# QueensGambit/CrazyAra

Hardware: AMD Instinct MI355X
Metric: nn_evals_per_sec (higher is better)
Workload: dtype f16x3; 1 GPU; crazyhouse RISEv2 19-block (34x8x8 planes -> 5184 policy + value), batch=256, inputs resident in HBM, random-init seeded weights; batch=256, parallelism=replicas x1, precision=float16x3

## Files before the change

### crazyara_amd/csrc/nn/kernels.h

```cpp
#pragma once
#include <hip/hip_runtime.h>
#include <cstdint>

namespace cra {

typedef _Float16 half_t;

constexpr int kSquares = 64;

inline int64_t packed_weight_elems(int cout_pad, int k_total) { return int64_t(cout_pad) * k_total; }

struct ConvArgs {
    const void* x;
    const void* wpk;
    const void* wpk_lo;
    const float* bias;
    const void* resid;
    void* out;
    int batch;
    int cin;
    int cout_pad;
    int cout_real;
    int cout_ld;
    int ks;
    int relu;
    int out_policy_f32;
    int out_flat;
    int flat_pitch;
    int out_rows_f32;
    int rows_valid;
    float* softmax_out;
    const float* planes;
    int planes_c;
    int p8;
    float acc_scale;
    const void *pre_wpk, *pre_wpk_lo;
    const float* pre_bias;
    float pre_acc_scale;
    int dev;
    int few_boards;
    int x_ld;
};

template <typename T> void launch_conv_gemm(const ConvArgs& a, hipStream_t s);

struct BlockArgs {
    const void* x;
    void* y;
    const void* w1pk;
    const float* b1;
    const float* wdw;
    const float* b2;
    const void* w3pk;
    const void* w1pk_lo;
    const void* w3pk_lo;
    const float* b3;
    int batch, C, cop_pad, ks;
    const float* gate;
    float* pool_out;
    const float* dwpk;
};
template <typename T> void launch_block(const BlockArgs& a, hipStream_t s);
void launch_conv_gemm_x3(const ConvArgs& a, hipStream_t s);
void launch_block_x3(const BlockArgs& a, hipStream_t s);
void init_x3_kernel_attributes();
int block_x3_chunk_channels();
struct X3TowerBlock {
    const void *w1pk, *w1pk_lo, *w3pk, *w3pk_lo;
    const float* dwpk;
    const float* b3;
    const float* se_w1t;
    const float* se_w2t;
    const float* se_b;
    int cop_pad;
    int se_kind;
    float w1_inv, w3_scale, w3_inv;
    int tail;
};
static_assert(sizeof(X3TowerBlock) == 96, "the tower kernels index a device array of these");
struct X3TowerArgs {
    const float* x;
    float* y;
    const X3TowerBlock* blocks;
    int nblocks;
    int batch;
    int p8;
    int ks;
    int symmetric;
    int no_tail;
    int no_quad;
};
void launch_tower_x3(const X3TowerArgs& a, hipStream_t s);
const char* tower_x3_kernel_name(const X3TowerArgs& a);
void launch_tower_x3_tail(const X3TowerArgs& a, hipStream_t s);
void init_x3_tail_kernel_attributes();
void launch_tower_x3_quad(const X3TowerArgs& a, hipStream_t s);
void init_x3_quad_kernel_attributes();
bool block_x3w_supports(int C, int ks);
void launch_block_x3w(const BlockArgs& a, hipStream_t s);
void init_x3_wblock_kernel_attributes();
void launch_se_gate_w(const float* pool, float* gate, int kind, const float* w1t, const float* w2t, const float* b1, int batch, int C, hipStream_t s);
constexpr int kX3WSplitMaxG = 8;
struct X3WSplitArgs {
    BlockArgs blk;
    const float* x_parts;
    float* y_parts;
    int gin, G;
    int stream_in;
};
int x3w_split_chunks(int cop_pad);
int x3w_split_shares(int cop_pad, int boards, int cu_count);
void launch_block_x3w_split(const X3WSplitArgs& a, hipStream_t s);
void launch_x3w_split_finish(const float* parts, int gin, float* y, float* pool_out, int batch, int C, hipStream_t s);
void init_x3_wsplit_kernel_attributes();
struct X3WTowerBlock {
    const void *w1pk, *w1pk_lo, *w3pk, *w3pk_lo;
    const float* dwpk;
    const float* b3;
    int cop_pad, ks;
};
static_assert(sizeof(X3WTowerBlock) == 56, "tower_x3w_kernel indexes a device array of these");
struct X3WTowerArgs {
    const float* x;
    float* y;
    const X3WTowerBlock* blocks;
    int nblocks;
    const float* gate;
    float* pool_out;
    int batch, C;
};
bool tower_x3w_supports(int C, int ks);
void launch_tower_x3w(const X3WTowerArgs& a, hipStream_t s);
void init_x3_wtower_kernel_attributes();
struct NtbLayer {
    const void *wh, *wl;
    const float* bias;
};
struct NtbArgs {
    const float* x;
    float* y;
    int batch, C, D, M, H;
    NtbLayer patch, qkv, proj, projection, mhca, mhca_proj, mlp1, mlp2;
};
bool ntb_x3w_supports(int C, int D, int M, int H);
void launch_ntb_x3w(const NtbArgs& a, hipStream_t s);
void init_x3_wntb_kernel_attributes();
struct X3SplitArgs {
    X3TowerBlock blk;
    const float* x_parts;
    float* y_parts;
    int gin;
    int batch, G;
    const float* pool_in;
    float* pool_out;
    int dev;
};
void launch_block_x3_split(const X3SplitArgs& a, hipStream_t s);
void launch_x3_split_finish(const float* parts, int gin, float* y, int batch, hipStream_t s);
template <typename T> void init_block_kernel_attributes();
template <typename T> int block_chunk_channels();

constexpr int kTowerWindow = 16;
struct TowerBlockDesc {
    const float* b3;
    const float* s3;
    const void* se_w1;
    const void* se_w2;
    const float* se_b;
    int cop_pad;
    int ks;
    int se_kind;
    float qx_inv, qt_inv, escale;
};
// ... 164 lines not shown
```

### crazyara_amd/csrc/nn/precision.cpp

```cpp
#include <cstdlib>
#include <stdexcept>

#include "rise_net.h"

namespace cra {

namespace {
constexpr bool kX3ValueHeadOneLaunch = true;
}

RiseNet::DevSwitches::DevSwitches() {
    if (const char* e = getenv("CRA_X3_CONV_DEV")) conv_dev = atoi(e);
    device_graph = getenv("CRA_DEVICE_GRAPH") != nullptr;
    lane_graph = getenv("CRA_LANE_GRAPH") != nullptr;
    lane_no_graph = getenv("CRA_LANE_NO_GRAPH") != nullptr;
    predict_copy = getenv("CRA_PREDICT_COPY") != nullptr;
    predict_zero_copy = getenv("CRA_PREDICT_ZERO_COPY") != nullptr;
    if (const char* e = getenv("CRA_LANE_LAUNCHES")) lane_launches = e[0];
    lane_sync = getenv("CRA_LANE_SYNC") != nullptr;
    if (const char* e = getenv("CRA_X3_TOWER")) x3_symmetric = e[0] == 's';
    if (const char* e = getenv("CRA_X3_SPLIT_DEV")) x3_split_dev = atoi(e);
    no_small_path = getenv("CRA_NO_SMALL_PATH") != nullptr;
    if (const char* e = getenv("CRA_SMALL_BATCH_CONV_SPLIT")) small_conv_split = atoi(e);
    tower_trace = getenv("CRA_TOWER_TRACE") != nullptr;
    x3_value_one_launch = kX3ValueHeadOneLaunch;
    if (const char* e = getenv("CRA_X3_VALUE_HEAD")) x3_value_one_launch = e[0] == 'o';
    value_head_debug = getenv("CRA_VALUE_HEAD_DEBUG") != nullptr;
    if (const char* e = getenv("CRA_VALUE_HEAD_LDS_PAD")) value_head_lds_pad = atoi(e);
    if (const char* e = getenv("CRA_VALUE_HEAD_VARIANT")) value_head_variant = atoi(e);
    x3_no_head_chain = getenv("CRA_X3_NO_HEAD_CHAIN") != nullptr;
    x3_no_tail = getenv("CRA_X3_NO_TAIL") != nullptr;
    x3_no_quad = getenv("CRA_X3_NO_QUAD") != nullptr;
    small_batch_heads_apart = getenv("CRA_SMALL_BATCH_HEADS_APART") != nullptr;
}

Precision parse_precision(const std::string& precision) {
    Precision v;
    std::string prec = precision;
    auto strip = [&](const std::string& tag) {
        if (prec.size() <= tag.size() || prec.compare(prec.size() - tag.size(), tag.size(), tag) != 0) return false;
        prec.resize(prec.size() - tag.size());
        return true;
    };
    if (strip("-3k")) v.one_launch = false;
    if (strip("-8w")) v.thin_waves = true;
    if (strip("-1wg")) v.board_split = false;
    if (strip("-1b")) v.boards_per_wg = 1;
    else if (strip("-2b")) v.boards_per_wg = 2;
    if (strip("-wtower")) v.wtower = v.wnet = v.wblock = true;
    else if (strip("-wsplit")) v.wsplit = v.wnet = v.wblock = true;
    else if (strip("-wnet")) v.wnet = v.wblock = true;
    else if (strip("-wblock")) v.wblock = true;
    if (strip("-unfused")) v.fused = v.tower = false;
    else if (strip("-perblock")) v.tower = false;
    using M = Precision::Mode;
    static const std::pair<const char*, M> kModes[] = {
        {"float16", M::Float16},   {"fp16", M::Float16},     {"half", M::Float16},      {"int8", M::Int8},
        {"fp8", M::Fp8},           {"float8", M::Fp8},       {"float32", M::Float32},   {"fp32", M::Float32},
        {"float16x3", M::Float16x3}, {"fp16x3", M::Float16x3}, {"f16x3", M::Float16x3},
        {"float16p8", M::Float16p8}, {"fp16p8", M::Float16p8}, {"f16p8", M::Float16p8}};
    for (const auto& m : kModes)
        if (prec == m.first) {
            v.mode = m.second;
            if (v.wtower && !v.x3()) throw std::invalid_argument("`-wtower` is a float16x3 kernel family (float16x3-wtower | float16p8-wtower), got '" + precision + "'");
            if (v.wtower && !v.fused) throw std::invalid_argument("`-wtower` and `-unfused` exclude each other, got '" + precision + "'");
            if (v.wsplit && !v.x3()) throw std::invalid_argument("`-wsplit` is a float16x3 kernel family (float16x3-wsplit | float16p8-wsplit), got '" + precision + "'");
            if (v.wsplit && !v.fused) throw std::invalid_argument("`-wsplit` and `-unfused` exclude each other, got '" + precision + "'");
            if (v.wsplit && !v.board_split)
                throw std::invalid_argument("`-wsplit` and `-1wg` exclude each other (several workgroups per board against one), got '" + precision + "'");
            if (v.wnet && !v.x3()) throw std::invalid_argument("`-wnet` is a float16x3 kernel family (float16x3-wnet | float16p8-wnet), got '" + precision + "'");
            if (v.wnet && !v.fused) throw std::invalid_argument("`-wnet` and `-unfused` exclude each other, got '" + precision + "'");
            if (v.wblock && !v.x3()) throw std::invalid_argument("`-wblock` is a float16x3 kernel family (float16x3-wblock | float16p8-wblock), got '" + precision + "'");
            if (v.wblock && !v.fused) throw std::invalid_argument("`-wblock` and `-unfused` exclude each other, got '" + precision + "'");
            return v;
        }
    throw std::invalid_argument("unsupported precision '" + precision + "' (float16 | float16x3 | float16p8 | float32 | fp8 | int8)");
}

}
```

### crazyara_amd/csrc/nn/rise_net.h

```cpp
#pragma once
#include <hip/hip_runtime.h>
#include <memory>
#include <string>
#include <utility>
#include <vector>

#include "board_net.h"
#include "netfile.h"

namespace cra {

uint8_t float_to_e4m3(float v);
uint8_t float_to_e5m2(float v);

struct Precision {
    enum class Mode { Float32, Float16, Float16x3, Float16p8, Fp8, Int8 };
    Mode mode = Mode::Float16;
    bool fused = true;
    bool tower = true;
    bool one_launch = true;
    bool thin_waves = false;
    bool board_split = true;
    bool wblock = false;
    bool wnet = false;
// ... 27 lines not shown
        const int* board_of = nullptr;
        int n = 0;
        int layout = 0;
        const void* descs = nullptr;
        const float* planes = nullptr;
        const uint16_t* idx = nullptr;
        const uint32_t* cnt = nullptr;
        uint32_t stride = 0;
        float* gathered = nullptr;
        float* probs = nullptr;
        float* logits = nullptr;
        float* value = nullptr;
        float* aux = nullptr;
    };
    void run_group(const Group& g);

    std::vector<std::pair<float, float>> calibration_maxima(const float* planes_host, int n_boards);

    void keep_logits(bool on) override;
    void* enable_block_dump(int* n_tiles);
    void dev_launch_op(int op, int iters);
    float* value_head_debug() const { return value_head_dbg_; }
    int dev_screen_prepare();
    long dev_screen_run(int op, int launches, long* words);
    std::string dev_screen_info(int op) const;
    void forward_async();

    int launches_per_forward() const { return launches_; }
    const char* op_name(int i) const;
    const char* op_kernel(int i) const;
    void time_ops(int iters, float* ms);
    float time_forward(int iters);

    struct IoOverride {
        const float* planes = nullptr;
        float* value = nullptr;
        float* probs = nullptr;
        float* aux = nullptr;
    };
    bool last_submit_was_zero_copy() const { return last_zero_copy_; }

private:
    friend class ExpertSet;
    struct ForwardCall {
        int boards = 0;
        const IoOverride* io = nullptr;
        int prev_g = 1;
    };
    RiseNet(const std::string& model_path, int device_id, int batch_size, const std::string& precision, const RiseNet* parent);
    struct Impl;
    template <typename T> struct Builder;
    template <typename T> void build(const NetFile& nf);
    template <typename T> void enqueue(hipStream_t s, ForwardCall call);
    template <typename T> void launch_op(int i, hipStream_t s, ForwardCall& call);
    void launch_forward_in_stream(ForwardCall call);
    void forward_on(hipStream_t s, ForwardCall call);
    int boards_of_call(int n_valid) const;
    void capture();
    bool buffers_are_pinned(const float* in_planes, float* value, float* probs, float* aux);
    bool last_zero_copy_ = false;
    bool counted_in_flight_ = false;
    int staged_calls_left_ = 0;
    struct DevSwitches {
        int conv_dev = -1;
        bool device_graph = false;
        bool lane_graph = false;
        bool lane_no_graph = false;
        bool predict_copy = false;
        bool predict_zero_copy = false;
        char lane_launches = 0;
        bool lane_sync = false;
        bool x3_symmetric = false;
        int x3_split_dev = 0;
        bool no_small_path = false;
        int small_conv_split = 2;
        bool tower_trace = false;
        bool x3_value_one_launch;
        bool value_head_debug = false;
        int value_head_lds_pad = -1;
        int value_head_variant = 0;
        bool x3_no_head_chain = false;
        bool x3_no_tail = false;
        bool x3_no_quad = false;
        bool small_batch_heads_apart = false;
        DevSwitches();
    } dev_;
    float* value_head_dbg_ = nullptr;

    std::string model_file_path_;
    Precision prec_;
    std::vector<std::pair<float, float>> int8_calib_;
    static constexpr int kBoardSplitMaxBatch = 64;
    std::unique_ptr<RiseNet> small_;
    bool owns_stream_ = true;
    int stream_slot_ = -1;
    std::string precision_arg_;
    int cu_count_ = 256;
    int launches_ = 0;
    hipGraph_t graph_ = nullptr;
    hipGraphExec_t graph_exec_ = nullptr;
    void* d_desc_ = nullptr;
    std::unique_ptr<Impl> impl_;
};

std::string int8_calibration_path(const std::string& model_file_path);
std::vector<std::pair<float, float>> read_int8_calibration(const std::string& model_file_path);
std::string calibrate_int8(const std::string& model_path, int device_id, const float* planes_host, int n_boards);
std::vector<float> default_calibration_planes(int channels, int version, int* n_boards);

}
```

### crazyara_amd/csrc/nn/rise_net_build.hip

```cpp
#include <algorithm>
#include <cmath>
#include <cstring>
#include <type_traits>

#include "../chess/planes_host.h"
#include "pack.h"
#include "rise_net_impl.h"

namespace cra {

namespace {
enum class Family {
    Tower,
    X3Tower,
    X3Split,
    Fused,
    WBlock,
    WSplit,
    WTower,
    Layers,
    Transformer,
    WNtb
};
struct BlockPlan {
// ... 645 lines not shown
    ++wntb_ops;
    prod_op = -1;
    std::swap(cur, nxt);
}

template <typename T> void RiseNet::Builder<T>::flush_tower() {
    if (tower_blocks.empty()) return;
    Op op;
    op.kind = OpKind::Tower;
    op.tw.x = cur;
    op.tw.y = nxt;
    op.tw.blocks = im.upload(tower_blocks);
    op.tw.nblocks = int(tower_blocks.size());
    const TowerImage ti = close_tower_streams(std::move(tower_streams), prec.fp8_tower());
    tower_streams = TowerStreams();
    if (prec.fp8_tower()) {
        op.tw.fp8 = prec.int8() ? 2 : 1;
        op.tw.wstream_e_frags = ti.e_frags;
        op.tw.wstream = im.upload(ti.w8);
    } else {
        op.tw.wstream = im.upload(ti.w);
    }
    op.tw.bstream = im.upload(ti.b);
    op.tw.pstream = im.upload(ti.p);
    op.tw.wstream_wave_frags = ti.w_wave_frags;
    op.tw.bstream_wave_floats = ti.b_wave_floats;
    op.tw.pstream_wave_bytes = ti.p_wave_bytes;
    op.tw.batch = B;
    op.tw.gate_in = tower_gate;
    if (dev.tower_trace) op.tw.trace = static_cast<unsigned long long*>(im.dalloc(2 * 256 * sizeof(unsigned long long)));
    prod_op = int(im.ops.size());
    im.ops.push_back(op);
    tower_blocks.clear();
    tower_gate = nullptr;
    std::swap(cur, nxt);
}

template <typename T> void RiseNet::Builder<T>::flush_x3_run() {
    if (x3_blocks.empty()) return;
    if (x3_split && x3_run_ks == 3) {
        if (!split_parts[0])
            for (auto& q : split_parts) q = static_cast<float*>(im.dalloc(size_t(B) * kSplitMaxG * kSquares * C * sizeof(float)));
        const int max_g = std::max(1, std::min(int(kSplitMaxG), net.cu_count_ / B));
        const int nb = int(x3_blocks.size());
        int gin = 1;
        for (int k = 0; k < nb; ++k) {
            Op op;
            op.kind = OpKind::BlockX3Split;
            op.xs.blk = x3_blocks[k];
            op.xs.x_parts = k == 0 ? reinterpret_cast<const float*>(cur) : split_parts[k % 2];
            op.xs.y_parts = split_parts[(k + 1) % 2];
            op.xs.gin = gin;
            op.xs.batch = B;
            op.xs.G = std::min(max_g, x3_blocks[k].cop_pad / block_x3_chunk_channels());
            op.xs.dev = dev.x3_split_dev;
            if (k > 0 && x3_blocks[k].se_kind != 0 && !(dev.x3_split_dev & 8)) {
                float* pools = static_cast<float*>(im.dalloc(size_t(B) * kSplitMaxG * C * sizeof(float)));
                im.ops.back().xs.pool_out = pools;
                op.xs.pool_in = pools;
            }
            gin = op.xs.G;
            im.ops.push_back(op);
        }
        Op fin;
        fin.kind = OpKind::X3SplitFinish;
        fin.xs.x_parts = split_parts[nb % 2];
        fin.xs.gin = gin;
        fin.xs.batch = B;
        fin.xs_y = reinterpret_cast<float*>(nxt);
        im.ops.push_back(fin);
    } else {
        Op op;
        op.kind = OpKind::TowerX3;
        op.tx.x = reinterpret_cast<const float*>(cur);
        op.tx.y = reinterpret_cast<float*>(nxt);
        op.tx.blocks = im.upload(x3_blocks);
        op.tx.nblocks = int(x3_blocks.size());
        op.tx.batch = B;
        op.tx.p8 = prec.p8() ? 1 : 0;
        op.tx.ks = x3_run_ks;
        op.tx.symmetric = dev.x3_symmetric ? 1 : 0;
        op.tx.no_tail = dev.x3_no_tail ? 1 : 0;
        op.tx.no_quad = dev.x3_no_quad ? 1 : 0;
        im.ops.push_back(op);
    }
    x3_blocks.clear();
    prod_op = -1;
    std::swap(cur, nxt);
}

template <typename T> void RiseNet::Builder<T>::one_launch_head() {
    const Folded fv = fold_bn(nf, "value_head.body.0", "value_head.body.1");
    const HeadStreams hs = pack_head(fold_bn(nf, "policy_head.body.0", "policy_head.body.1"), fold_bn(nf, "policy_head.body.3", ""), fv, C, cv, cp);
    Op op;
    op.kind = OpKind::Head;
    HeadArgs& h = op.hd;
    h.x = cur;
    h.logits = net.d_logits_;
    h.probs = net.d_probs_;
    h.value = net.d_value_;
    h.aux = net.d_aux_;
    h.s1 = im.upload(hs.s1);
    h.b1 = im.upload(hs.b1);
    h.s2 = im.upload(hs.s2);
    h.s1_wave_frags = 9 * 16 + 16 + 16;
    h.s2_wave_frags = 18 * 3 + 9;
    h.vconv_bias = im.upload_d2f(fv.b, 8);
    h.cp = cp;
    h.batch = B;
    if (dev.tower_trace) h.trace = static_cast<unsigned long long*>(im.dalloc(64 * sizeof(unsigned long long)));
    const int nfl = kSquares * cv;
    if (wdl) {
        h.fc1_w = im.upload(pack_value_wdl(nf, nfl, 512));
        const float* bw = nf.get("value_head.body_wdl.0.bias").data;
        h.wdl_b[0] = bw[0]; h.wdl_b[1] = bw[1]; h.wdl_b[2] = bw[2];
        h.wdl_b[3] = nf.get("value_head.body_plys.0.bias").data[0];
        h.wdlp = 1;
        macs += 4.0 * nfl;
    } else {
        const TensorView& w2 = nf.get("value_head.body_final.2.weight");
        const float* bb = nf.get("value_head.body_final.0.bias").data;
        h.fc1_w = im.upload(pack_value_fc1_threads(nf, nfl, fc));
        h.fc1_b = im.upload(std::vector<float>(bb, bb + fc));
        h.fc2_w = im.upload(std::vector<float>(w2.data, w2.data + fc));
        h.fc2_b = nf.get("value_head.body_final.2.bias").data[0];
        macs += double(nfl) * fc + fc;
    }
    macs += double(kSquares) * 9 * (double(C) * C + double(C) * cp) + double(kSquares) * C * cv;
    im.ops.push_back(op);
}

template <typename T> void RiseNet::Builder<T>::policy_head() {
    const bool head_chain = prec.p8() && policy_map && C == 256 && round_up(cp, 16) <= 128 && !x3_split;
    const bool head_chain_x3 = prec.x3() && !prec.p8() && prec.fused && policy_map && C == 256 && round_up(cp, 16) <= 128 && !x3_split &&
                               !dev.x3_no_head_chain;
    if (head_chain || head_chain_x3) {
        Folded f1 = fold_bn(nf, "policy_head.body.0", "policy_head.body.1");
        double inv1 = 1.0;
        SplitPack s1 = head_chain ? pack_dense_p8(f1, C, C, 3, C, C, &inv1) : pack_dense_split(f1, C, C, 3, C, C);
        add_conv("policy_head.body.3", "", cur, nullptr, nullptr, C, C, cp, 3, false, net.d_logits_, head_chain);
        ConvArgs& c = im.ops.back().conv;
        c.pre_wpk = im.upload(s1.hi);
        c.pre_wpk_lo = im.upload(s1.lo);
        c.pre_bias = im.upload_d2f(f1.b, C);
        c.pre_acc_scale = float(inv1);
        macs += double(kSquares) * C * C * 9;
        return;
    }
    add_conv("policy_head.body.0", "policy_head.body.1", cur, nxt, nullptr, C, C, C, 3, true, nullptr, !x3_split);
    im.ops.back().conv.few_boards = x3_split ? dev.small_conv_split : 0;
    if (policy_map) {
        add_conv("policy_head.body.3", "", nxt, nullptr, nullptr, C, C, cp, 3, false, net.d_logits_, !x3_split);
        return;
    }
    const int nfl = cp * kSquares, Bpad = round_up(B, 64);
    T* pflat = static_cast<T*>(im.dalloc(size_t(Bpad) * nfl * sizeof(T)));
    HIP_CHECK(hipMemset(pflat, 0, size_t(Bpad) * nfl * sizeof(T)));
    ConvArgs& c1 = conv_op(fold_bn(nf, "policy_head.body.3", "policy_head.body2.0"), nxt, pflat, C, C, cp, 3, 1);
    c1.out_flat = 1;
    c1.flat_pitch = nfl;
    macs += double(kSquares) * C * cp * 9;
    const TensorView& w = nf.get("policy_head.body3.0.weight");
    const float* bb = nf.get("policy_head.body3.0.bias").data;
    Folded fl;
    fl.w.assign(w.data, w.data + size_t(n_labels) * nfl);
    fl.b.assign(bb, bb + n_labels);
// ... 177 lines not shown
```

### crazyara_amd/csrc/nn/x3.hip

```cpp
#include "kernels.h"
#include "device_utils.h"
#include "value_head_body.h"
#include "x3_device.h"

#include <algorithm>
#include <cstdlib>
#include <stdexcept>
#include <type_traits>

#ifndef X3_SGB_VALU
#define X3_SGB_VALU 10
#endif

namespace cra {

namespace {

typedef int i32x4_x3 __attribute__((ext_vector_type(4)));
typedef int i32x8_x3 __attribute__((ext_vector_type(8)));
__device__ __forceinline__ uint32_t x3_high_bytes(uint32_t p01, uint32_t p23) {
    return __builtin_amdgcn_perm(p23, p01, 0x07050301u);
}
__device__ __forceinline__ void split4_b8(const float (&v)[4], half4& hi, uint32_t& h8, uint32_t& l8) {
    uint32_t h[2], l[2];
// ... 1894 lines not shown
                for (int t = 0; t < 4; ++t) {
                    const char* pp = pj + (kk & 1) * 64 * T8ROW + t * 16 * T8ROW;
                    b8[t] = x3_cat(*reinterpret_cast<const half8*>(pp), *reinterpret_cast<const half8*>(pp + 32));
                }
            };
            const int knext = kk + 1 < n ? kk + 1 : kk;
            read_h(0);
            read_8(0);
#pragma unroll
            for (int s2 = 0; s2 < CK / 32; ++s2) {
                if (s2 + 1 < CK / 32) read_h(s2 + 1);
                __builtin_amdgcn_sched_barrier(0);
#pragma unroll
                for (int j = 0; j < NJ; ++j)
#pragma unroll
                    for (int t = 0; t < 4; ++t) x3_mfma(p_h[s2 & 1][j], bh[s2 & 1][t], accX[j][t], !(X3_ABL & 4));
                if (s2 & 1) {
#pragma unroll
                    for (int j = 0; j < NJ; ++j)
#pragma unroll
                        for (int t = 0; t < 4; ++t) x3_mfma8(p_8[j], b8[t], accX[j][t], !(X3_ABL & 4));
                    __builtin_amdgcn_sched_barrier(0);
                    if (s2 == 1) { read_8(1); load_p8(kk, 1); } else load_p8(knext, 0);
                }
                if (s2 + 2 < CK / 32) load_ph(kk, s2 + 2); else load_ph(knext, s2 + 2 - CK / 32);
                __builtin_amdgcn_sched_barrier(0);
            }
            X3_STAMP(10);
            if (kk + 1 < n) __syncthreads();
            X3_STAMP(11);
        }
        {
            const float pi = d.w3_inv;
#pragma unroll
            for (int j = 0; j < NJ; ++j)
#pragma unroll
                for (int t = 0; t < 4; ++t) accX[j][t] *= pi;
        }
        const bool next_gated = blk + 1 < a.nblocks && a.blocks[blk + 1].se_kind != 0;
        if (!next_gated) write_tiles();
        { const int kk = n; X3_STAMP(12); }
        __syncthreads();
        { const int kk = n; X3_STAMP(13); }
    }
    float* yb = a.y + size_t(b) * 64 * C;
#pragma unroll
    for (int j = 0; j < NJ; ++j)
#pragma unroll
        for (int t = 0; t < 4; ++t)
            *reinterpret_cast<f32x4*>(yb + size_t(x3_square(t * 16 + l15)) * C + (w * NJ + j) * 16 + lg * 4) = accX[j][t];
}

void init_x3_kernel_attributes() {
    (void)hipFuncSetAttribute(reinterpret_cast<const void*>(&block_x3_kernel), hipFuncAttributeMaxDynamicSharedMemorySize, int(X3Block::lds_bytes));
    (void)hipFuncSetAttribute(reinterpret_cast<const void*>(&tower_x3_kernel), hipFuncAttributeMaxDynamicSharedMemorySize, int(X3Block::lds_bytes));
    (void)hipFuncSetAttribute(reinterpret_cast<const void*>(&block_x3_split_kernel), hipFuncAttributeMaxDynamicSharedMemorySize, int(X3Block::lds_bytes));
    (void)hipFuncSetAttribute(reinterpret_cast<const void*>(&tower_x3_roles_kernel<3>), hipFuncAttributeMaxDynamicSharedMemorySize, int(X3Block::lds_bytes));
    (void)hipFuncSetAttribute(reinterpret_cast<const void*>(&tower_x3_roles_kernel<5>), hipFuncAttributeMaxDynamicSharedMemorySize, int(X3Block::lds_bytes + 8192));
    init_x3_tail_kernel_attributes();
    init_x3_quad_kernel_attributes();
    (void)hipFuncSetAttribute(reinterpret_cast<const void*>(&tower_p8_kernel<3>), hipFuncAttributeMaxDynamicSharedMemorySize, int(X3Block::lds_bytes));
    (void)hipFuncSetAttribute(reinterpret_cast<const void*>(&tower_p8_kernel<5>), hipFuncAttributeMaxDynamicSharedMemorySize, int(X3Block::lds_bytes + 8192));
    (void)hipFuncSetAttribute(reinterpret_cast<const void*>(&conv3x3_x3_chain_kernel), hipFuncAttributeMaxDynamicSharedMemorySize, int(ConvX3::lds_bytes));
    const int conv_p8_lds = int(ConvP8::lds_bytes);
    (void)hipFuncSetAttribute(reinterpret_cast<const void*>(&conv3x3_p8_chain_kernel), hipFuncAttributeMaxDynamicSharedMemorySize, conv_p8_lds);
    (void)hipFuncSetAttribute(reinterpret_cast<const void*>(&conv3x3_p8_kernel<2, 8>), hipFuncAttributeMaxDynamicSharedMemorySize, conv_p8_lds);
    (void)hipFuncSetAttribute(reinterpret_cast<const void*>(&conv3x3_p8_kernel<1, 8>), hipFuncAttributeMaxDynamicSharedMemorySize, conv_p8_lds);
}
int block_x3_chunk_channels() { return X3Block::CK; }

void launch_block_x3(const BlockArgs& a, hipStream_t s) {
    hipLaunchKernelGGL(block_x3_kernel, dim3(a.batch), dim3(X3Block::NTHR), X3Block::lds_bytes, s, a);
}
void launch_block_x3_split(const X3SplitArgs& a, hipStream_t s) {
    const int n = a.blk.cop_pad / X3Block::CK;
    if (a.G < 1 || a.G > n || a.G > 16 || a.gin < 1 || a.gin > 16) throw std::invalid_argument("block_x3_split: 1 <= G <= min(chunks, 16), 1 <= gin <= 16");
    hipLaunchKernelGGL(block_x3_split_kernel, dim3(8 * a.G * ((a.batch + 7) / 8)), dim3(X3Block::NTHR), X3Block::lds_bytes, s, a);
}
void launch_x3_split_finish(const float* parts, int gin, float* y, int batch, hipStream_t s) {
    const int n4 = batch * 64 * X3Block::C / 4;
    hipLaunchKernelGGL(x3_split_finish_kernel, dim3(std::min(1024, (n4 + 255) / 256)), dim3(256), 0, s, parts, gin, y, batch);
}
namespace {
enum class X3TowerKernel { P8_5, P8_3, Quad3, Tail5, Tail3, Roles5, Roles3, Symmetric };
X3TowerKernel pick_tower_x3(const X3TowerArgs& a) {
    const bool symmetric = a.symmetric != 0;
    if (a.p8) {
        if (symmetric) throw std::invalid_argument("Precision float16p8 runs the two-role tower only");
        return a.ks == 5 ? X3TowerKernel::P8_5 : X3TowerKernel::P8_3;
    }
    if (!symmetric && !a.no_tail) {
        if (a.ks == 5) return X3TowerKernel::Tail5;
        return a.no_quad ? X3TowerKernel::Tail3 : X3TowerKernel::Quad3;
    }
    if (a.ks == 5) return X3TowerKernel::Roles5;
    return symmetric ? X3TowerKernel::Symmetric : X3TowerKernel::Roles3;
}
}
const char* tower_x3_kernel_name(const X3TowerArgs& a) {
    switch (pick_tower_x3(a)) {
        case X3TowerKernel::P8_5: return "tower_p8_kernel<5>";
        case X3TowerKernel::P8_3: return "tower_p8_kernel<3>";
        case X3TowerKernel::Quad3: return "tower_x3_quad_kernel<3>";
        case X3TowerKernel::Tail5: return "tower_x3_tail_kernel<5>";
        case X3TowerKernel::Tail3: return "tower_x3_tail_kernel<3>";
        case X3TowerKernel::Roles5: return "tower_x3_roles_kernel<5>";
        case X3TowerKernel::Roles3: return "tower_x3_roles_kernel<3>";
        case X3TowerKernel::Symmetric: return "tower_x3_kernel";
    }
    return "?";
}
void launch_tower_x3(const X3TowerArgs& a, hipStream_t s) {
    switch (pick_tower_x3(a)) {
        case X3TowerKernel::P8_5: hipLaunchKernelGGL(tower_p8_kernel<5>, dim3(a.batch), dim3(X3Block::NTHR), X3Block::lds_bytes + 8192, s, a); break;
        case X3TowerKernel::P8_3: hipLaunchKernelGGL(tower_p8_kernel<3>, dim3(a.batch), dim3(X3Block::NTHR), X3Block::lds_bytes, s, a); break;
        case X3TowerKernel::Quad3: launch_tower_x3_quad(a, s); break;
        case X3TowerKernel::Tail5:
        case X3TowerKernel::Tail3: launch_tower_x3_tail(a, s); break;
        case X3TowerKernel::Roles5: hipLaunchKernelGGL(tower_x3_roles_kernel<5>, dim3(a.batch), dim3(X3Block::NTHR), X3Block::lds_bytes + 8192, s, a); break;
        case X3TowerKernel::Roles3: hipLaunchKernelGGL(tower_x3_roles_kernel<3>, dim3(a.batch), dim3(X3Block::NTHR), X3Block::lds_bytes, s, a); break;
        case X3TowerKernel::Symmetric: hipLaunchKernelGGL(tower_x3_kernel, dim3(a.batch), dim3(X3Block::NTHR), X3Block::lds_bytes, s, a); break;
    }
}

}
```

### crazyara_amd/csrc/nn/x3_quad.cpp

```cpp
#include "x3_device.h"
#include "x3_quad.h"

#include <type_traits>

namespace cra {

template <int KS>
__global__ __launch_bounds__(512) void tower_x3_quad_kernel(const X3TowerArgs a) {
    static_assert(KS == 3, "depthwise 3x3 (X3DepthwiseQuad); 5x5 runs stay on tower_x3_tail_kernel");
    constexpr int REC = 256;
    using G = X3Block;
    static_assert(G::NE == 1 && G::T2BUF == 2 && G::CK == 128, "the role kernel uses the NE = 1 tile geometry (two t2 buffers of 128 channels)");
    static_assert(X3Q_T2T_HALVES <= 64 * G::TROW, "t2T of a chunk lies in the [64][TROW] tile's place");
    constexpr int C = G::C, CK = G::CK, XROW = G::XROW, TROW = G::TROW;
    extern __shared__ __attribute__((aligned(16))) char smem[];
    const X3Tiles T = x3_tiles(smem);
    const int b = blockIdx.x;
    const int tid = threadIdx.x, lane = tid & 63, l15 = lane & 15, lg = lane >> 4;
    const int wave = __builtin_amdgcn_readfirstlane(tid >> 6);
    const bool expand_role = wave < 4;
    const int w = wave & 3;
    const uint32_t lane_off = uint32_t(lane) * 16u;
    x3_stage_tile(T, a.x + size_t(b) * 64 * C, nullptr, tid);
    __syncthreads();
    constexpr int EW = 2;
    half8 e_h[EW][2], e_l[EW][2];
    bool first_chunk_requested = false;
    if (expand_role) {
    for (int blk = 0; blk < a.nblocks; ++blk) {
        const X3TowerBlock& d = a.blocks[blk];
        if (blk > 0 && d.se_kind != 0) {
            x3_se_gate_from_mean(d, reinterpret_cast<float*>(T.t2h), tid);
            __syncthreads();
            first_chunk_requested = false;
#pragma unroll
            for (int ne = 0; ne < 2; ++ne) {
#pragma unroll
                for (int q = 0; q < EW; ++q) { asm volatile("" : "=v"(e_h[q][ne])); asm volatile("" : "=v"(e_l[q][ne])); }
            }
        }
        const X3Weights W = x3_weights(d.w1pk, d.w1pk_lo, d.w3pk, d.w3pk_lo, d.dwpk, d.cop_pad);
        const int n = W.cop_pad / CK;
        const bool tail = __builtin_amdgcn_readfirstlane(d.tail) != 0;
#ifdef CRA_X3_TRACE
        const bool tracing = (b == 0 || b == 131) && blk == CRA_X3_TRACE;
        int trace_n = 0;
#endif
        {
            const X3QuadOffsets qo = x3_quad_offsets(lane);
            int sto[4];
#pragma unroll
            for (int t = 0; t < 4; ++t) sto[t] = x3q_store_offset(0, l15, lg, t);
            auto e_tile = [&](int i, int ne) { return i * (CK / 16) + (tail && i == n - 1 ? w : w * 2 + ne); };
            auto load_e = [&](auto one_c, int i, int s) {
                if constexpr (X3_ABL & 16) return;
#pragma unroll
                for (int ne = 0; ne < (decltype(one_c)::value ? 1 : 2); ++ne) {
                    const uint32_t f = uint32_t(e_tile(i, ne)) * (C / 32) + uint32_t(s);
                    e_h[s % EW][ne] = x3_frag(W.w1h, lane_off, f);
                    e_l[s % EW][ne] = x3_frag(W.w1l, lane_off, f);
                }
            };
            auto load_first_chunk = [&](const X3Weights& Wx, bool one) {
                if constexpr (X3_ABL & 16) return;
#pragma unroll
                for (int s = 0; s < EW; ++s)
#pragma unroll
                    for (int ne = 0; ne < 2; ++ne) {
                        const uint32_t f = uint32_t(one ? w : w * 2 + ne) * (C / 32) + uint32_t(s);
                        e_h[s][ne] = x3_frag(Wx.w1h, lane_off, f);
                        e_l[s][ne] = x3_frag(Wx.w1l, lane_off, f);
                    }
            };
            if constexpr (X3_ABL & 16) {
#pragma unroll
                for (int s = 0; s < EW; ++s)
#pragma unroll
                    for (int ne = 0; ne < 2; ++ne) e_h[s][ne] = e_l[s][ne] = *reinterpret_cast<const half8*>(T.xh + lane * 8);
            }
            if (!first_chunk_requested) load_first_chunk(W, tail && n == 1);
            float* const my_dws = T.dws + (w * 2) * REC;
            f32x4 accE[2][4], accD[2][4];
            X3DepthwiseQuad dw;
            auto interval = [&](auto hase_c, auto hasd_c, auto onee_c, auto oned_c, int i) {
                constexpr bool HASE = decltype(hase_c)::value, HASD = decltype(hasd_c)::value;
                constexpr bool ONEE = decltype(onee_c)::value, ONED = decltype(oned_c)::value;
                static_assert(!(ONEE && !HASE) && !(ONED && (HASE || !HASD)), "the tail chunk is expanded in interval n - 1 and runs the depthwise alone in interval n");
                constexpr int NEE = ONEE ? 1 : 2;
                half8 ring_h[4], ring_l[4];
                auto read_step = [&](int st) {
// ... 35 lines not shown
                            if (st + 3 < 4 * (C / 32)) read_step(st + 3);
#pragma unroll
                            for (int ne = 0; ne < NEE; ++ne) {
                                x3_mfma(ring_h[st % 4], e_l[sl % EW][ne], accE[ne][t], !(X3_ABL & 2));
                                x3_mfma(ring_l[st % 4], e_h[sl % EW][ne], accE[ne][t], !(X3_ABL & 2));
                                x3_mfma(ring_h[st % 4], e_h[sl % EW][ne], accE[ne][t], !(X3_ABL & 2));
                            }
                        }
                        if (sl + EW < C / 32) load_e(onee_c, i, sl + EW);
                        else if constexpr (ONEE) load_e(onee_c, i, sl + EW - C / 32);
                        else load_e(onee_c, i + 1 < n ? i + 1 : i, sl + EW - C / 32);
                    }
                    if constexpr (HASD) {
                        if (ph == 0) dw.gather(accD[dt], lg, qo);
                        if (ph == 1) { dw.template taps_rank<0>(); dw.template taps_rank<1>(); dw.template pin_rank<0>(); dw.template pin_rank<1>(); }
                        if (ph == 2) { dw.template taps_rank<2>(); dw.template taps_rank<3>(); dw.template pin_rank<2>(); dw.template pin_rank<3>(); }
                        if (ph == 3) {
                            const int tile = ONED ? w : w * 2 + dt;
#pragma unroll
                            for (int t = 0; t < 4; ++t) {
                                half4 h, l;
                                split4(dw.outv[t], h, l);
                                if constexpr (X3_ABL & 64) {
                                    asm volatile("" ::"v"(h), "v"(l));
                                } else {
                                    *reinterpret_cast<half4*>(t2h + tile * 16 * X3Q_T2T_ROW + sto[t]) = h;
                                    *reinterpret_cast<half4*>(t2l + tile * 16 * X3Q_T2T_ROW + sto[t]) = l;
                                }
                            }
                        }
                    }
                    if constexpr (HASE && HASD) {
#pragma unroll
                        for (int r = 0; r < 12 * NEE; ++r) {
                            __builtin_amdgcn_sched_group_barrier(0x008, 1, 0);
                            __builtin_amdgcn_sched_group_barrier(0x002, ONEE ? 8 : 4, 0);
                        }
                    }
                    __builtin_amdgcn_sched_barrier(0);
                }
                if constexpr (HASE) {
#pragma unroll
                    for (int ne = 0; ne < NEE; ++ne)
#pragma unroll
                        for (int h2 = 0; h2 < REC / 256; ++h2) *reinterpret_cast<f32x4*>(my_dws + ne * REC + h2 * 256 + lane * 4) = dw_raw[ne][h2];
#pragma unroll
                    for (int ne = 0; ne < NEE; ++ne)
#pragma unroll
                        for (int t = 0; t < 4; ++t) accD[ne][t] = accE[ne][t];
                }
            };
            constexpr std::true_type yes{};
            constexpr std::false_type no{};
            auto run = [&](auto hase_c, auto hasd_c, auto onee_c, auto oned_c, int i) {
                const int kk = i - 1;
                X3_STAMP(0);
                interval(hase_c, hasd_c, onee_c, oned_c, i);
                X3_STAMP(3);
                if constexpr (!(X3_ABL & 32)) __syncthreads();
                X3_STAMP(4);
            };
            const int nfull = tail ? n - 1 : n;
            if (nfull == 0) run(yes, no, yes, no, 0);
            else run(yes, no, no, no, 0);
            for (int i = 1; i < nfull; ++i) run(yes, yes, no, no, i);
            if (tail) {
                if (nfull > 0) run(yes, yes, yes, no, n - 1);
                run(no, yes, no, yes, n);
            } else run(no, yes, no, no, n);
            first_chunk_requested = false;
            if (blk + 1 < a.nblocks && a.blocks[blk + 1].se_kind == 0) {
                const X3TowerBlock& dn = a.blocks[blk + 1];
                load_first_chunk(x3_weights(dn.w1pk, dn.w1pk_lo, dn.w3pk, dn.w3pk_lo, dn.dwpk, dn.cop_pad), dn.tail != 0 && dn.cop_pad == CK);
                first_chunk_requested = true;
            }
            __syncthreads();
            { const int kk = n; X3_STAMP(5); }
        }
    }
    } else {
    constexpr int NJ = 4;
    f32x4 accX[NJ][4];
    x3_stream_load<NJ>(accX, a.x + size_t(b) * 64 * C, w * NJ, l15, lg);
    for (int blk = 0; blk < a.nblocks; ++blk) {
        const X3TowerBlock& d = a.blocks[blk];
        if (blk > 0 && d.se_kind != 0) x3_stream_se<NJ>(T, d, accX, reinterpret_cast<float*>(T.t2h), w * NJ, tid);
        const X3Weights W = x3_weights(d.w1pk, d.w1pk_lo, d.w3pk, d.w3pk_lo, d.dwpk, d.cop_pad);
        const int n = W.cop_pad / CK;
        const int nslab3 = W.cop_pad >> 5;
        const bool tail = __builtin_amdgcn_readfirstlane(d.tail) != 0;
#ifdef CRA_X3_TRACE
        const bool tracing = (b == 0 || b == 131) && blk == CRA_X3_TRACE;
        int trace_n = 0;
#endif
        {
            constexpr int PW = 2;
            half8 p_h[PW][NJ], p_l[PW][NJ];
            int rdo[2][4];
#pragma unroll
            for (int hh = 0; hh < 2; ++hh)
#pragma unroll
                for (int t = 0; t < 4; ++t) rdo[hh][t] = x3q_read_offset(0, hh, t, l15, lg);
            auto load_p = [&](int k, int s2) {
                if constexpr (X3_ABL & 16) return;
#pragma unroll
                for (int j = 0; j < NJ; ++j) {
                    const uint32_t f = uint32_t(w * NJ + j) * uint32_t(nslab3) + uint32_t(k * (CK / 32) + s2);
                    p_h[s2 % PW][j] = x3_frag(W.w3h, lane_off, f);
                    p_l[s2 % PW][j] = x3_frag(W.w3l, lane_off, f);
                }
            };
            if constexpr (X3_ABL & 16) {
#pragma unroll
                for (int s2 = 0; s2 < PW; ++s2)
#pragma unroll
                    for (int j = 0; j < NJ; ++j) p_h[s2][j] = p_l[s2][j] = *reinterpret_cast<const half8*>(T.xl + lane * 8);
            }
            x3_stream_add_bias<NJ>(accX, d.b3, w * NJ, lg);
#pragma unroll
            for (int s2 = 0; s2 < PW; ++s2) load_p(0, s2);
            if constexpr (!(X3_ABL & 32)) {
                __syncthreads();
                __syncthreads();
            }
            auto project = [&](auto one_c, int kk) {
                constexpr int NS2 = decltype(one_c)::value ? CK / 64 : CK / 32;
                const half_t* const t2h = T.t2h + (kk & 1) * 64 * TROW;
                const half_t* const t2l = T.t2l + (kk & 1) * 64 * TROW;
                const half_t* rd[2][4];
#pragma unroll
                for (int hh = 0; hh < 2; ++hh)
#pragma unroll
                    for (int t = 0; t < 4; ++t) rd[hh][t] = t2h + rdo[hh][t];
                const int to_lo = int(t2l - t2h);
                X3_STAMP(8);
                half8 bh[2][4], bl[2][4];
                auto read_t2 = [&](int s2, half8 (&h)[4], half8 (&l)[4]) {
#pragma unroll
                    for (int t = 0; t < 4; ++t) {
                        if constexpr (X3_ABL & 8) {
                            h[t] = p_h[s2 % PW][0];
                            l[t] = p_l[s2 % PW][0];
                        } else {
                            h[t] = x3q_read_fragment(rd[0][t] + s2 * 32 * X3Q_T2T_ROW, rd[1][t] + s2 * 32 * X3Q_T2T_ROW);
                            l[t] = x3q_read_fragment(rd[0][t] + s2 * 32 * X3Q_T2T_ROW + to_lo, rd[1][t] + s2 * 32 * X3Q_T2T_ROW + to_lo);
                        }
                    }
                };
                read_t2(0, bh[0], bl[0]);
#pragma unroll
                for (int s2 = 0; s2 < NS2; ++s2) {
                    if (s2 + 1 < NS2) read_t2(s2 + 1, bh[(s2 + 1) & 1], bl[(s2 + 1) & 1]);
                    __builtin_amdgcn_sched_barrier(0);
#pragma unroll
                    for (int j = 0; j < NJ; ++j)
#pragma unroll
                        for (int t = 0; t < 4; ++t) x3_mfma(p_l[s2 % PW][j], bh[s2 & 1][t], accX[j][t], !(X3_ABL & 4));
#pragma unroll
                    for (int j = 0; j < NJ; ++j)
#pragma unroll
                        for (int t = 0; t < 4; ++t) x3_mfma(p_h[s2 % PW][j], bl[s2 & 1][t], accX[j][t], !(X3_ABL & 4));
#pragma unroll
                    for (int j = 0; j < NJ; ++j)
#pragma unroll
                        for (int t = 0; t < 4; ++t) x3_mfma(p_h[s2 % PW][j], bh[s2 & 1][t], accX[j][t], !(X3_ABL & 4));
                    if (s2 + PW < NS2) load_p(kk, s2 + PW);
                    else if constexpr (decltype(one_c)::value) load_p(kk, s2 + PW - NS2);
                    else load_p(kk + 1 < n ? kk + 1 : kk, s2 + PW - NS2);
                    if (s2 == 1) X3_STAMP(9);
                    __builtin_amdgcn_sched_barrier(0);
                }
                X3_STAMP(10);
            };
            const int nfull = tail ? n - 1 : n;
            for (int kk = 0; kk < nfull; ++kk) {
                project(std::false_type{}, kk);
                if (kk + 1 < n) {
                    if constexpr (!(X3_ABL & 32)) __syncthreads();
                }
                X3_STAMP(11);
            }
            if (tail) {
                const int kk = n - 1;
                project(std::true_type{}, kk);
                X3_STAMP(11);
            }
            if (blk + 1 < a.nblocks && a.blocks[blk + 1].se_kind == 0) x3_stream_write_tiles<NJ>(T, accX, w * NJ, l15, lg);
            { const int kk = n; X3_STAMP(12); }
            __syncthreads();
            { const int kk = n; X3_STAMP(13); }
        }
    }
    x3_stream_store<NJ>(accX, a.y + size_t(b) * 64 * C, w * NJ, l15, lg);
    }
}

void init_x3_quad_kernel_attributes() {
    (void)hipFuncSetAttribute(reinterpret_cast<const void*>(&tower_x3_quad_kernel<3>), hipFuncAttributeMaxDynamicSharedMemorySize, int(X3Block::lds_bytes));
}
void launch_tower_x3_quad(const X3TowerArgs& a, hipStream_t s) {
    hipLaunchKernelGGL(tower_x3_quad_kernel<3>, dim3(a.batch), dim3(X3Block::NTHR), X3Block::lds_bytes, s, a);
}

}
```

Baseline: 365,100 evals/s.

## Write next-block input tiles interleaved with the last projection MFMAs in quad tower

Adds an EARLY_TILES variant of the quad tower kernel, on by default. The last projection slab runs as a 'seam' step that splits each finished accumulator tile to hi/lo halves and writes it to LDS between MFMA groups, instead of a separate write-tiles pass after the loop. The intent is to hide the LDS tile writes behind MFMA latency and shorten the per-block serial tail. Empty asm is used to recompute lane indices so fewer registers stay live. It adds scheduling complexity, and it always writes tiles, even when the next block is an SE block or there is no next block.

```diff
diff --git a/crazyara_amd/csrc/nn/kernels.h b/crazyara_amd/csrc/nn/kernels.h
--- a/crazyara_amd/csrc/nn/kernels.h
+++ b/crazyara_amd/csrc/nn/kernels.h
@@ -89,6 +89,7 @@
     int symmetric;
     int no_tail;
     int no_quad;
+    int no_early_tiles;
 };
 void launch_tower_x3(const X3TowerArgs& a, hipStream_t s);
 const char* tower_x3_kernel_name(const X3TowerArgs& a);
diff --git a/crazyara_amd/csrc/nn/precision.cpp b/crazyara_amd/csrc/nn/precision.cpp
--- a/crazyara_amd/csrc/nn/precision.cpp
+++ b/crazyara_amd/csrc/nn/precision.cpp
@@ -31,6 +31,7 @@
     x3_no_head_chain = getenv("CRA_X3_NO_HEAD_CHAIN") != nullptr;
     x3_no_tail = getenv("CRA_X3_NO_TAIL") != nullptr;
     x3_no_quad = getenv("CRA_X3_NO_QUAD") != nullptr;
+    x3_no_early_tiles = getenv("CRA_X3_NO_EARLY_TILES") != nullptr;
     small_batch_heads_apart = getenv("CRA_SMALL_BATCH_HEADS_APART") != nullptr;
 }
 
diff --git a/crazyara_amd/csrc/nn/rise_net.h b/crazyara_amd/csrc/nn/rise_net.h
--- a/crazyara_amd/csrc/nn/rise_net.h
+++ b/crazyara_amd/csrc/nn/rise_net.h
@@ -133,6 +133,7 @@
         bool x3_no_head_chain = false;
         bool x3_no_tail = false;
         bool x3_no_quad = false;
+        bool x3_no_early_tiles = false;
         bool small_batch_heads_apart = false;
         DevSwitches();
     } dev_;
diff --git a/crazyara_amd/csrc/nn/rise_net_build.hip b/crazyara_amd/csrc/nn/rise_net_build.hip
--- a/crazyara_amd/csrc/nn/rise_net_build.hip
+++ b/crazyara_amd/csrc/nn/rise_net_build.hip
@@ -751,6 +751,7 @@
         op.tx.symmetric = dev.x3_symmetric ? 1 : 0;
         op.tx.no_tail = dev.x3_no_tail ? 1 : 0;
         op.tx.no_quad = dev.x3_no_quad ? 1 : 0;
+        op.tx.no_early_tiles = dev.x3_no_early_tiles ? 1 : 0;
         im.ops.push_back(op);
     }
     x3_blocks.clear();
diff --git a/crazyara_amd/csrc/nn/x3.hip b/crazyara_amd/csrc/nn/x3.hip
--- a/crazyara_amd/csrc/nn/x3.hip
+++ b/crazyara_amd/csrc/nn/x3.hip
@@ -2000,7 +2000,7 @@
     hipLaunchKernelGGL(x3_split_finish_kernel, dim3(std::min(1024, (n4 + 255) / 256)), dim3(256), 0, s, parts, gin, y, batch);
 }
 namespace {
-enum class X3TowerKernel { P8_5, P8_3, Quad3, Tail5, Tail3, Roles5, Roles3, Symmetric };
+enum class X3TowerKernel { P8_5, P8_3, Quad3, Quad3Late, Tail5, Tail3, Roles5, Roles3, Symmetric };
 X3TowerKernel pick_tower_x3(const X3TowerArgs& a) {
     const bool symmetric = a.symmetric != 0;
     if (a.p8) {
@@ -2009,7 +2009,7 @@
     }
     if (!symmetric && !a.no_tail) {
         if (a.ks == 5) return X3TowerKernel::Tail5;
-        return a.no_quad ? X3TowerKernel::Tail3 : X3TowerKernel::Quad3;
+        return a.no_quad ? X3TowerKernel::Tail3 : a.no_early_tiles ? X3TowerKernel::Quad3Late : X3TowerKernel::Quad3;
     }
     if (a.ks == 5) return X3TowerKernel::Roles5;
     return symmetric ? X3TowerKernel::Symmetric : X3TowerKernel::Roles3;
@@ -2020,6 +2020,7 @@
         case X3TowerKernel::P8_5: return "tower_p8_kernel<5>";
         case X3TowerKernel::P8_3: return "tower_p8_kernel<3>";
         case X3TowerKernel::Quad3: return "tower_x3_quad_kernel<3>";
+        case X3TowerKernel::Quad3Late: return "tower_x3_quad_kernel<3> late-tiles";
         case X3TowerKernel::Tail5: return "tower_x3_tail_kernel<5>";
         case X3TowerKernel::Tail3: return "tower_x3_tail_kernel<3>";
         case X3TowerKernel::Roles5: return "tower_x3_roles_kernel<5>";
@@ -2032,7 +2033,8 @@
     switch (pick_tower_x3(a)) {
         case X3TowerKernel::P8_5: hipLaunchKernelGGL(tower_p8_kernel<5>, dim3(a.batch), dim3(X3Block::NTHR), X3Block::lds_bytes + 8192, s, a); break;
         case X3TowerKernel::P8_3: hipLaunchKernelGGL(tower_p8_kernel<3>, dim3(a.batch), dim3(X3Block::NTHR), X3Block::lds_bytes, s, a); break;
-        case X3TowerKernel::Quad3: launch_tower_x3_quad(a, s); break;
+        case X3TowerKernel::Quad3:
+        case X3TowerKernel::Quad3Late: launch_tower_x3_quad(a, s); break;
         case X3TowerKernel::Tail5:
         case X3TowerKernel::Tail3: launch_tower_x3_tail(a, s); break;
         case X3TowerKernel::Roles5: hipLaunchKernelGGL(tower_x3_roles_kernel<5>, dim3(a.batch), dim3(X3Block::NTHR), X3Block::lds_bytes + 8192, s, a); break;
diff --git a/crazyara_amd/csrc/nn/x3_quad.cpp b/crazyara_amd/csrc/nn/x3_quad.cpp
--- a/crazyara_amd/csrc/nn/x3_quad.cpp
+++ b/crazyara_amd/csrc/nn/x3_quad.cpp
@@ -5,7 +5,7 @@
 
 namespace cra {
 
-template <int KS>
+template <int KS, bool EARLY_TILES>
 __global__ __launch_bounds__(512) void tower_x3_quad_kernel(const X3TowerArgs a) {
     static_assert(KS == 3, "depthwise 3x3 (X3DepthwiseQuad); 5x5 runs stay on tower_x3_tail_kernel");
     constexpr int REC = 256;
@@ -207,9 +207,13 @@
     constexpr int NJ = 4;
     f32x4 accX[NJ][4];
     x3_stream_load<NJ>(accX, a.x + size_t(b) * 64 * C, w * NJ, l15, lg);
+    auto own = [](int v) {
+        if constexpr (EARLY_TILES) asm volatile("" : "+v"(v));
+        return v;
+    };
     for (int blk = 0; blk < a.nblocks; ++blk) {
         const X3TowerBlock& d = a.blocks[blk];
-        if (blk > 0 && d.se_kind != 0) x3_stream_se<NJ>(T, d, accX, reinterpret_cast<float*>(T.t2h), w * NJ, tid);
+        if (blk > 0 && d.se_kind != 0) x3_stream_se<NJ>(T, d, accX, reinterpret_cast<float*>(T.t2h), w * NJ, own(tid));
         const X3Weights W = x3_weights(d.w1pk, d.w1pk_lo, d.w3pk, d.w3pk_lo, d.dwpk, d.cop_pad);
         const int n = W.cop_pad / CK;
         const int nslab3 = W.cop_pad >> 5;
@@ -241,22 +245,33 @@
 #pragma unroll
                     for (int j = 0; j < NJ; ++j) p_h[s2][j] = p_l[s2][j] = *reinterpret_cast<const half8*>(T.xl + lane * 8);
             }
-            x3_stream_add_bias<NJ>(accX, d.b3, w * NJ, lg);
+            x3_stream_add_bias<NJ>(accX, d.b3, w * NJ, EARLY_TILES ? (own(tid) >> 4) & 3 : lg);
 #pragma unroll
             for (int s2 = 0; s2 < PW; ++s2) load_p(0, s2);
             if constexpr (!(X3_ABL & 32)) {
                 __syncthreads();
                 __syncthreads();
             }
-            auto project = [&](auto one_c, int kk) {
-                constexpr int NS2 = decltype(one_c)::value ? CK / 64 : CK / 32;
+            auto seam_tile = [&](int ln, int j, int t) {
+                const float v[4] = {accX[j][t][0], accX[j][t][1], accX[j][t][2], accX[j][t][3]};
+                half4 h, l;
+                split4(v, h, l);
+                const int at = (t * 16 + (ln & 15)) * XROW + (w * NJ + j) * 16 + (ln >> 4) * 4;
+                *reinterpret_cast<half4*>(T.xh + at) = h;
+                *reinterpret_cast<half4*>(T.xl + at) = l;
+            };
+            auto project = [&](auto one_c, auto seam_c, int kk) {
+                constexpr bool SEAM = decltype(seam_c)::value;
+                constexpr int NS2 = SEAM ? 2 : decltype(one_c)::value ? CK / 64 : CK / 32;
+                constexpr int NREAD = SEAM ? 4 : NS2;
                 const half_t* const t2h = T.t2h + (kk & 1) * 64 * TROW;
                 const half_t* const t2l = T.t2l + (kk & 1) * 64 * TROW;
+                const int ln = own(tid) & 63;
                 const half_t* rd[2][4];
 #pragma unroll
                 for (int hh = 0; hh < 2; ++hh)
 #pragma unroll
-                    for (int t = 0; t < 4; ++t) rd[hh][t] = t2h + rdo[hh][t];
+                    for (int t = 0; t < 4; ++t) rd[hh][t] = t2h + (EARLY_TILES ? x3q_read_offset(0, hh, t, ln & 15, ln >> 4) : rdo[hh][t]);
                 const int to_lo = int(t2l - t2h);
                 X3_STAMP(8);
                 half8 bh[2][4], bl[2][4];
@@ -273,9 +288,10 @@
                     }
                 };
                 read_t2(0, bh[0], bl[0]);
+                if (!SEAM || !tail) {
 #pragma unroll
                 for (int s2 = 0; s2 < NS2; ++s2) {
-                    if (s2 + 1 < NS2) read_t2(s2 + 1, bh[(s2 + 1) & 1], bl[(s2 + 1) & 1]);
+                    if (s2 + 1 < NREAD) read_t2(s2 + 1, bh[(s2 + 1) & 1], bl[(s2 + 1) & 1]);
                     __builtin_amdgcn_sched_barrier(0);
 #pragma unroll
                     for (int j = 0; j < NJ; ++j)
@@ -289,42 +305,78 @@
                     for (int j = 0; j < NJ; ++j)
 #pragma unroll
                         for (int t = 0; t < 4; ++t) x3_mfma(p_h[s2 % PW][j], bh[s2 & 1][t], accX[j][t], !(X3_ABL & 4));
-                    if (s2 + PW < NS2) load_p(kk, s2 + PW);
+                    if (s2 + PW < NREAD) load_p(kk, s2 + PW);
                     else if constexpr (decltype(one_c)::value) load_p(kk, s2 + PW - NS2);
                     else load_p(kk + 1 < n ? kk + 1 : kk, s2 + PW - NS2);
                     if (s2 == 1) X3_STAMP(9);
                     __builtin_amdgcn_sched_barrier(0);
                 }
-                X3_STAMP(10);
-            };
+                }
+                if constexpr (SEAM) {
+                    if (tail) read_t2(1, bh[1], bl[1]);
+                    else read_t2(3, bh[1], bl[1]);
+                    __builtin_amdgcn_sched_barrier(0);
+#pragma unroll
+                    for (int j = 0; j < NJ; ++j) {
+#pragma unroll
+                        for (int m = 0; m < 24; ++m) {
+                            const int q = m / 12, term = (m / 4) % 3, t = m % 4;
+                            x3_mfma(term == 0 ? p_l[q][j] : p_h[q][j], term == 1 ? bl[q][t] : bh[q][t], accX[j][t], !(X3_ABL & 4));
+                            if (m % 6 == 5 && j > 0) {
+                                __builtin_amdgcn_sched_barrier(0);
+                                seam_tile(ln, j - 1, m / 6);
+                                __builtin_amdgcn_sched_barrier(0);
+                            }
+                        }
+                        if (j == 1) { if (tail) X3_STAMP(9); }
+                    }
+                    X3_STAMP(10);
+                    mfma_retire(accX[NJ - 1][0], accX[NJ - 1][1], accX[NJ - 1][2], accX[NJ - 1][3]);
+#pragma unroll
+                    for (int t = 0; t < 4; ++t) seam_tile(ln, NJ - 1, t);
+                } else {
+                    X3_STAMP(10);
+                }
+            };
+            constexpr std::false_type steady{};
             const int nfull = tail ? n - 1 : n;
-            for (int kk = 0; kk < nfull; ++kk) {
-                project(std::false_type{}, kk);
+            const int nsteady = EARLY_TILES ? n - 1 : nfull;
+            for (int kk = 0; kk < nsteady; ++kk) {
+                project(std::false_type{}, steady, kk);
                 if (kk + 1 < n) {
                     if constexpr (!(X3_ABL & 32)) __syncthreads();
                 }
                 X3_STAMP(11);
             }
-            if (tail) {
+            if constexpr (EARLY_TILES) {
                 const int kk = n - 1;
-                project(std::true_type{}, kk);
+                project(std::false_type{}, std::true_type{}, kk);
                 X3_STAMP(11);
-            }
-            if (blk + 1 < a.nblocks && a.blocks[blk + 1].se_kind == 0) x3_stream_write_tiles<NJ>(T, accX, w * NJ, l15, lg);
+            } else if (tail) {
+                const int kk = n - 1;
+                project(std::true_type{}, steady, kk);
+                X3_STAMP(11);
+            }
+            if constexpr (!EARLY_TILES) {
+                if (blk + 1 < a.nblocks && a.blocks[blk + 1].se_kind == 0) x3_stream_write_tiles<NJ>(T, accX, w * NJ, l15, lg);
+            }
             { const int kk = n; X3_STAMP(12); }
             __syncthreads();
             { const int kk = n; X3_STAMP(13); }
         }
     }
-    x3_stream_store<NJ>(accX, a.y + size_t(b) * 64 * C, w * NJ, l15, lg);
+    const int lane_y = own(tid) & 63;
+    x3_stream_store<NJ>(accX, a.y + size_t(b) * 64 * C, w * NJ, lane_y & 15, lane_y >> 4);
     }
 }
 
 void init_x3_quad_kernel_attributes() {
-    (void)hipFuncSetAttribute(reinterpret_cast<const void*>(&tower_x3_quad_kernel<3>), hipFuncAttributeMaxDynamicSharedMemorySize, int(X3Block::lds_bytes));
+    (void)hipFuncSetAttribute(reinterpret_cast<const void*>(&tower_x3_quad_kernel<3, true>), hipFuncAttributeMaxDynamicSharedMemorySize, int(X3Block::lds_bytes));
+    (void)hipFuncSetAttribute(reinterpret_cast<const void*>(&tower_x3_quad_kernel<3, false>), hipFuncAttributeMaxDynamicSharedMemorySize, int(X3Block::lds_bytes));
 }
 void launch_tower_x3_quad(const X3TowerArgs& a, hipStream_t s) {
-    hipLaunchKernelGGL(tower_x3_quad_kernel<3>, dim3(a.batch), dim3(X3Block::NTHR), X3Block::lds_bytes, s, a);
+    if (a.no_early_tiles) hipLaunchKernelGGL((tower_x3_quad_kernel<3, false>), dim3(a.batch), dim3(X3Block::NTHR), X3Block::lds_bytes, s, a);
+    else hipLaunchKernelGGL((tower_x3_quad_kernel<3, true>), dim3(a.batch), dim3(X3Block::NTHR), X3Block::lds_bytes, s, a);
 }
 
 }
```

Result: no change. 364,900 evals/s (-0.0%).
